# gillesdegottex/percivaltts

Measured on AMD Instinct MI355X. Metric: acoustic frames/sec per WGAN-GP critic+gen step, higher is better.
Workload: dtype f32

## Files before the change

### include/percival_hip.h

```cpp
#ifndef PERCIVAL_HIP_H
#define PERCIVAL_HIP_H

#include <stddef.h>
#include <stdint.h>

#ifdef __cplusplus
extern "C" {
#endif

#define PTTS_OK            0
#define PTTS_EINVAL       -1
#define PTTS_ELAUNCH      -2
#define PTTS_EWORKSPACE   -3
#define PTTS_EDEVICE      -4

#define PTTS_IN_NONE     0
#define PTTS_IN_LRELU    1
#define PTTS_IN_MASKMUL  2

#define PTTS_PAD_SAME    0
#define PTTS_PAD_CAUSAL  1

#define PTTS_ACT_NONE    0
#define PTTS_ACT_LRELU   1
#define PTTS_ACT_SIGMOID 2
#define PTTS_ACT_TANH    3

const char* ptts_version(void);
const char* ptts_device_arch(void);
const char* ptts_last_error(void);
int ptts_device_status(unsigned* word_out);
int ptts_device_status_clear(void);
unsigned* ptts_device_status_word(void);
int ptts_device_status_message(unsigned word, char* buf, size_t n);
int ptts_set_deterministic(int on);
int ptts_get_deterministic(void);
int ptts_set_bf16_products(int on);
int ptts_get_bf16_products(void);

int ptts_conv2d_fwd(const float* x, const float* w, const float* bias ,
                    const float* in_scale , const float* in_shift ,
                    const float* mask_src ,
                    float* y,
                    int B, int T, int F, int Cin, int Cout, int KT, int KF,
                    int dil_t, int pad_mode, int in_mode, float alpha, void* stream);

size_t ptts_conv2d_bwd_workspace_bytes(int B, int T, int F, int Cin, int Cout, int KT, int KF, int dil_t);
int ptts_conv2d_bwd(const float* dy, const float* x, const float* w,
                    const float* in_scale, const float* in_shift, const float* mask_src,
                    float* dx, float* dw, float* dbias, float* dscale, float* dshift,
                    void* workspace, size_t workspace_bytes,
                    int B, int T, int F, int Cin, int Cout, int KT, int KF,
                    int dil_t, int pad_mode, int in_mode, float alpha, void* stream);

int ptts_conv2d_bwd_partials(const float* dy, const float* x, const float* w, const float* mask_src,
                             float* dx, void* workspace, size_t workspace_bytes, int* nblocks_out,
                             int B, int T, int F, int Cin, int Cout, int KT, int KF,
                             int dil_t, int pad_mode, int in_mode, float alpha, void* stream);
typedef struct ptts_conv2d_reduce_desc {
    const float* partials;
    int nblocks, npart, nw, cout;
    float* dw; float* dbias;
} ptts_conv2d_reduce_desc;
int ptts_conv2d_reduce_grouped(const ptts_conv2d_reduce_desc* descs, int n, void* stream);

int ptts_conv2d_wide_supported(int F, int Cin, int Cout, int KT, int KF, int dil_t);
int ptts_conv2d_wide_fwd(const float* x, const float* w, const float* bias, const float* in_scale, const float* in_shift,
                         const float* mask_src, float* y, int B, int T, int F, int Cin, int Cout, int KT, int KF,
                         int dil_t, int pad_mode, int in_mode, float alpha, void* stream);
size_t ptts_conv2d_wide_bwd_workspace_bytes(int B, int T, int F, int Cin, int Cout, int KT, int KF, int dil_t);
int ptts_conv2d_wide_bwd_partials(const float* dy, const float* x, const float* w, const float* in_scale, const float* in_shift,
                                  const float* mask_src, float* dx, void* workspace, size_t workspace_bytes,
                                  int* nblocks_out, int* npart_out, int want_dw, int want_affine,
                                  int B, int T, int F, int Cin, int Cout, int KT, int KF,
                                  int dil_t, int pad_mode, int in_mode, float alpha, void* stream);

int ptts_conv2d_mfma_supported(int F, int Cin, int Cout, int KT, int KF, int dil_t);
size_t ptts_conv2d_mfma_table_bytes(int KT);
int ptts_conv2d_mfma_tables(const float* w, void* table_fwd, void* table_bwd, int KT, int KF, int Cin, int Cout,
                            int planes , void* stream);
int ptts_conv2d_mfma_tables_grouped(const float* const* w, void* const* table_fwd, void* const* table_bwd, int n, int planes,
                                    void* stream);
int ptts_conv2d_mfma_fwd(const void* x, const void* table, const float* bias, const float* in_scale, const float* in_shift,
                         const void* mask_src, const void* out_mask, void* y,
                         int B, int T, int F, int KT, int dil_t, int pad_t, int in_mode, float alpha,
                         int planes, int in_bf16, int out_bf16, void* stream);
int ptts_conv2d_mfma_fwd_stats_supported(int F, int dil_t, int in_mode);
int ptts_conv2d_mfma_fwd_stats(const float* x, const void* table, const float* bias, const float* in_scale, const float* in_shift,
                               float* y, int B, int T, int F, int KT, int pad_t, int in_mode, float alpha,
                               double* stats, int capacity_rows, int* nrows_out, void* stream);
size_t ptts_conv2d_mfma_wgrad_workspace_bytes(int B, int T);
int ptts_conv2d_mfma_wgrad_partials(const void* dy, const void* x, const void* mask_src, void* workspace,
                                    size_t workspace_bytes, int* nblocks_out, int* npart_out, int B, int T, int F,
                                    int KT, int dil_t, int pad_t, int in_mode, float alpha,
                                    int planes, int x_bf16, int dy_bf16, void* stream);
size_t ptts_conv2d_mfma_bwd_fused_workspace_bytes(int B, int T);
int ptts_conv2d_mfma_bwd_fused_supported(int F, int dil_t, int planes);
int ptts_conv2d_mfma_bwd_fused(const void* p, const void* q, const void* mask_src, const void* table, void* y,
                               void* workspace, size_t workspace_bytes, int* nblocks_out, int* npart_out,
                               int B, int T, int F, int KT, int pad_t, int kind, float alpha, void* stream);
int ptts_conv2d_mfma_bwd_fused_affine(const float* p, const float* q, const void* table, float* y, void* workspace, size_t workspace_bytes,
                                      int* nblocks_out, int* npart_out, int B, int T, int F, int KT, int pad_t, float alpha,
                                      const float* q_scale, const float* q_shift, void* stream);
int ptts_conv2d_mfma_debug(int flags, void* stamp_buf);

int ptts_conv2d_chain_supported(int F, int L, int Cin0, int C, int KT, int KF);
int ptts_conv2d_chain_blocks(int F, int L, int* origin, int* own_lo, int* own_hi, int cap);
int ptts_conv2d_chain_debug(void* stamp_buf);
size_t ptts_conv2d_chain_tables_bytes(void);
size_t ptts_conv2d_chain_partials_bytes(int L);
long long ptts_conv2d_chain_map_elems(int B, int T, int F);
int ptts_conv2d_chain_tables(const float* const* w, const float* const* b, void* tables, int L, int cin0, void* stream);
int ptts_conv2d_chain_fwd(const float* x0, long long ldx, const void* tables, void* maps, void* a_last,
                          int B, int T, int F, int L, float alpha, void* stream);
int ptts_conv2d_chain_bwd(const void* d_last, int d_bf16, const float* x0, long long ldx, const void* maps, const void* a_last,
                          const void* tables, float* partials, size_t partials_bytes, int* nblocks_out, int* npart_out,
                          int B, int T, int F, int L, int cin0, float alpha, void* stream);
int ptts_conv2d_chain_bwd_data(const void* d_last, int d_bf16, const void* maps, const void* a_last, const void* tables,
                               void* gmaps, float* g0, int B, int T, int F, int L, float alpha, void* stream);
int ptts_conv2d_chain_second(const float* u0, const void* gmaps, const void* maps, const void* a_last, const void* tables,
                             void* out, int out_bf16, float* partials, size_t partials_bytes, int* nblocks_out, int* npart_out,
                             int B, int T, int F, int L, int cin0, float alpha, void* stream);

int ptts_gemm(const float* A, const float* Bm, const float* bias, float* C,
              int M, int N, int K,
              int transA, long long lda, long long rows_per_seg, long long seg_stride,
              int transB, long long ldb, long long ldc,
              int in_mode, const float* in_scale, const float* in_shift, const float* mask_src,
              float alpha, int accumulate, const float* out_mask, float* colsum_b, void* stream);
// ... 370 lines not shown
```

### percivaltts_amd/csrc/conv2d.hip

```cpp
#include "common.h"
#include <cstdlib>

namespace ptts {

template <int C> struct VecIO;
template <> struct VecIO<1> {
    static __device__ __forceinline__ void ld(const float* p, float* v) { v[0] = p[0]; }
    static __device__ __forceinline__ void st(float* p, const float* v) { p[0] = v[0]; }
};
template <> struct VecIO<2> {
    static __device__ __forceinline__ void ld(const float* p, float* v) {
        float2 t = *reinterpret_cast<const float2*>(p); v[0] = t.x; v[1] = t.y; }
    static __device__ __forceinline__ void st(float* p, const float* v) {
        *reinterpret_cast<float2*>(p) = make_float2(v[0], v[1]); }
};
template <> struct VecIO<4> {
    static __device__ __forceinline__ void ld(const float* p, float* v) {
        float4 t = *reinterpret_cast<const float4*>(p); v[0] = t.x; v[1] = t.y; v[2] = t.z; v[3] = t.w; }
    static __device__ __forceinline__ void st(float* p, const float* v) {
        *reinterpret_cast<float4*>(p) = make_float4(v[0], v[1], v[2], v[3]); }
};

constexpr int CONV_THREADS = 256;

// ... 497 lines not shown
                    const float av = arow[(size_t)fq * CIN];
#pragma unroll
                    for (int kf = 0; kf < KF; ++kf) {
                        const int slot = (u + KF - 1 - kf) % KF;
                        if (PKO) {
#pragma unroll
                            for (int h = 0; h < HO; ++h)
                                accw2[kf][h] = pkfma(av, (f2){win[slot][2 * h], win[slot][2 * h + (PKO ? 1 : 0)]}, accw2[kf][h]);
                        } else {
#pragma unroll
                            for (int co = 0; co < COUT; ++co)
                                accw[kf][co] = fmaf(av, win[slot][co], accw[kf][co]);
                        }
                    }
                }
            }
        }
    }
    if (PKO) {
#pragma unroll
        for (int kf = 0; kf < KF; ++kf)
#pragma unroll
            for (int h = 0; h < HO; ++h) {
                accw[kf][2 * h] = accw2[kf][h].x;
                accw[kf][2 * h + (PKO ? 1 : 0)] = accw2[kf][h].y;
            }
    }
    float s_b[COUT];
#pragma unroll
    for (int co = 0; co < COUT; ++co) s_b[co] = 0.f;
    if (want_dw) {
        for (int idx = tid; idx < TT * F; idx += CONV_THREADS) {
            const int r = idx / F, f = idx - r * F;
            if (t0 + r >= T) break;
            float g[COUT];
            VecIO<COUT>::ld(dyt + ((size_t)(r + lo_t) * cols + f + LO_F) * COUT, g);
#pragma unroll
            for (int co = 0; co < COUT; ++co) s_b[co] += g[co];
        }
    }
    __syncthreads();

    float* red = smem;
    float* red2 = smem + (size_t)NGRP * NW;
    if (want_dw && grp < NGRP) {
#pragma unroll
        for (int kf = 0; kf < KF; ++kf)
#pragma unroll
            for (int co = 0; co < COUT; ++co)
                red[(size_t)grp * NW + ((rkt * KF + kf) * CIN + rci) * COUT + co] = accw[kf][co];
    }
    {
        const int wave = tid >> 6, lane = tid & 63;
#pragma unroll
        for (int co = 0; co < COUT; ++co) {
            const float v = wave_sum(s_b[co]);
            if (lane == 0) red2[wave * (COUT + 2 * CIN) + co] = v;
        }
#pragma unroll
        for (int ci = 0; ci < CIN; ++ci) {
            const float v1 = wave_sum(s_scale[ci]);
            const float v2 = wave_sum(s_shift[ci]);
            if (lane == 0) {
                red2[wave * (COUT + 2 * CIN) + COUT + ci] = v1;
                red2[wave * (COUT + 2 * CIN) + COUT + CIN + ci] = v2;
            }
        }
    }
    __syncthreads();
    float* out = partials + (size_t)(blockIdx.y * gridDim.x + blockIdx.x) * NPART;
    if (want_dw) {
        for (int j = tid; j < NW; j += CONV_THREADS) {
            float s = 0.f;
#pragma unroll
            for (int g = 0; g < NGRP; ++g) s += red[(size_t)g * NW + j];
            out[j] = s;
        }
    }
    if (tid < COUT + 2 * CIN) {
        float s = 0.f;
#pragma unroll
        for (int wv = 0; wv < CONV_THREADS / 64; ++wv) s += red2[wv * (COUT + 2 * CIN) + tid];
        out[NW + tid] = s;
    }
}

__global__ __launch_bounds__(256) void reduce_partials_kernel(const float* __restrict__ partials,
                                                              int nblocks, int npart,
                                                              float* __restrict__ dw, int nw,
                                                              float* __restrict__ dbias, int cout,
                                                              float* __restrict__ dscale,
                                                              float* __restrict__ dshift, int cin) {
    __shared__ double sh[4];
    const int j = blockIdx.x;
    double s = 0.0;
    for (int blk = threadIdx.x; blk < nblocks; blk += 256) s += (double)partials[(size_t)blk * npart + j];
    s = wave_sum(s);
    if ((threadIdx.x & 63) == 0) sh[threadIdx.x >> 6] = s;
    __syncthreads();
    if (threadIdx.x == 0) {
        const float v = (float)(sh[0] + sh[1] + sh[2] + sh[3]);
        if (j < nw) { if (dw) dw[j] = v; }
        else if (j < nw + cout) { if (dbias) dbias[j - nw] = v; }
        else if (j < nw + cout + cin) { if (dscale) dscale[j - nw - cout] = v; }
        else { if (dshift) dshift[j - nw - cout - cin] = v; }
    }
}

__device__ __forceinline__ float gen_in(const float* __restrict__ x, const float* __restrict__ in_scale,
                                        const float* __restrict__ in_shift,
                                        const float* __restrict__ mask_src, long long off, int c,
                                        int in_mode, float alpha) {
    float v = x[off];
    if (in_mode == PTTS_IN_LRELU) {
        if (in_scale) v = v * in_scale[c] + in_shift[c];
        v = lrelu(v, alpha);
    } else if (in_mode == PTTS_IN_MASKMUL) {
        v *= lrelu_d(mask_src[off], alpha);
    }
    return v;
}

__global__ void conv2d_fwd_generic(const float* __restrict__ x, const float* __restrict__ w,
                                   const float* __restrict__ bias, const float* __restrict__ in_scale,
                                   const float* __restrict__ in_shift, const float* __restrict__ mask_src,
                                   float* __restrict__ y, long long total, int T, int F, int Cin, int Cout,
                                   int KT, int KF, int dil_t, int pad_t, int in_mode, float alpha) {
    const int PF = (KF - 1) / 2;
    for (long long i = blockIdx.x * (long long)blockDim.x + threadIdx.x; i < total;
         i += (long long)gridDim.x * blockDim.x) {
        const int co = (int)(i % Cout);
        long long pix = i / Cout;
        const int f = (int)(pix % F);
        pix /= F;
        const int t = (int)(pix % T);
        const long long b = pix / T;
        float acc = bias ? bias[co] : 0.f;
        for (int kt = 0; kt < KT; ++kt) {
            const int tt = t + kt * dil_t - pad_t;
            if (tt < 0 || tt >= T) continue;
            for (int kf = 0; kf < KF; ++kf) {
                const int ff = f + kf - PF;
                if (ff < 0 || ff >= F) continue;
                const long long base = ((b * T + tt) * F + ff) * Cin;
                for (int ci = 0; ci < Cin; ++ci)
                    acc = fmaf(gen_in(x, in_scale, in_shift, mask_src, base + ci, ci, in_mode, alpha),
                               w[((kt * KF + kf) * Cin + ci) * Cout + co], acc);
            }
        }
        y[i] = acc;
    }
}

__global__ void conv2d_bwd_dx_generic(const float* __restrict__ dy, const float* __restrict__ x,
                                      const float* __restrict__ w, const float* __restrict__ in_scale,
                                      const float* __restrict__ in_shift, float* __restrict__ dx,
                                      long long total, int T, int F, int Cin, int Cout, int KT, int KF,
                                      int dil_t, int pad_t, int in_mode, float alpha) {
    const int PF = (KF - 1) / 2;
    for (long long i = blockIdx.x * (long long)blockDim.x + threadIdx.x; i < total;
         i += (long long)gridDim.x * blockDim.x) {
        const int ci = (int)(i % Cin);
        long long pix = i / Cin;
        const int f = (int)(pix % F);
        pix /= F;
        const int t = (int)(pix % T);
// ... 159 lines not shown

#define PTTS_CONV_CASES(M)                                                                    \
    M(1, 1, 3, 3) M(1, 2, 3, 3) M(1, 4, 3, 3) M(2, 1, 3, 3) M(2, 2, 3, 3) M(2, 4, 3, 3)       \
    M(4, 1, 3, 3) M(4, 2, 3, 3) M(4, 4, 3, 3)                                                 \
    M(1, 1, 5, 5) M(1, 2, 5, 5) M(1, 4, 5, 5) M(2, 1, 5, 5) M(2, 2, 5, 5) M(2, 4, 5, 5)       \
    M(4, 1, 5, 5) M(4, 2, 5, 5) M(4, 4, 5, 5)

}

using namespace ptts;

extern "C" int ptts_conv2d_fwd(const float* x, const float* w, const float* bias, const float* in_scale,
                               const float* in_shift, const float* mask_src, float* y, int B, int T, int F,
                               int Cin, int Cout, int KT, int KF, int dil_t, int pad_mode, int in_mode,
                               float alpha, void* stream) {
    PTTS_REQUIRE(x && w && y, "conv2d_fwd: null tensor");
    PTTS_REQUIRE(B > 0 && T > 0 && F > 0 && Cin > 0 && Cout > 0 && KT > 0 && KF > 0 && dil_t > 0,
                 "conv2d_fwd: bad dims B=%d T=%d F=%d Cin=%d Cout=%d KT=%d KF=%d dil=%d", B, T, F, Cin, Cout, KT, KF, dil_t);
    PTTS_REQUIRE(in_mode >= 0 && in_mode <= 2, "conv2d_fwd: bad in_mode %d", in_mode);
    PTTS_REQUIRE((in_scale == nullptr) == (in_shift == nullptr), "conv2d_fwd: scale/shift must come together");
    PTTS_REQUIRE(in_mode != PTTS_IN_MASKMUL || mask_src, "conv2d_fwd: MASKMUL needs mask_src");
    PTTS_REQUIRE(B <= 65535, "conv2d_fwd: B too large");
    hipStream_t st = (hipStream_t)stream;
    const ConvGeom g = geom(KT, dil_t, pad_mode);
#define FWD_LAUNCH(CI, CO, KTT, KFF, NRR, MK)                                                           \
    hipLaunchKernelGGL((conv2d_fwd_kernel<CI, CO, KTT, KFF, NRR, MK>), dim3(grid), dim3(CONV_THREADS), lds, \
                       st, x, w, bias, in_scale, in_shift, mask_src, y, T, F, tl.TT, tl.ntiles,             \
                       tl.ntiles * B, dil_t, g.pad_t, in_mode, alpha)
#define FWD_CASE(CI, CO, KTT, KFF)                                                                       \
    if (Cin == CI && Cout == CO && KT == KTT && KF == KFF) {                                             \
        const int nspr = (F + KFF - 1) / KFF;                                                            \
        const int cols = nspr * KFF + KFF - 1;                                                           \
        const Tile tl = pick_tile_fwd(T, F, KTT, KFF, dil_t, cols);                                      \
        const int rows = tl.TT + (KTT - 1) * dil_t;                                                      \
        const size_t in_fl = ((size_t)rows * cols * CI + 3) & ~(size_t)3;                                \
        const size_t lds = (in_fl + (size_t)tl.TT * F * CO) * sizeof(float);                             \
        const int nr = (tl.TT * nspr + CONV_THREADS - 1) / CONV_THREADS;                                 \
        if (tl.TT > 0 && lds <= 150 * 1024 && nr <= 2 && rows * cols <= NPF * CONV_THREADS) {            \
            int per_cu = (int)((150 * 1024) / lds);                                                      \
            if (per_cu > 4) per_cu = 4;                                                                  \
            long long grid = (long long)tl.ntiles * B;                                                   \
            if (grid > 256LL * per_cu) grid = 256LL * per_cu;                                            \
            const bool mk = in_mode == PTTS_IN_MASKMUL;                                                  \
            if (conv_use_mfma() && dil_t >= 1) {                                                         \
                if (mk) hipLaunchKernelGGL((conv2d_fwd_mfma_kernel<CI, CO, KTT, KFF, true, 2>), dim3(grid), dim3(CONV_THREADS), lds, st, x, w, bias, in_scale, in_shift, mask_src, y, T, F, tl.TT, tl.ntiles, tl.ntiles * B, dil_t, g.pad_t, in_mode, alpha); \
                else hipLaunchKernelGGL((conv2d_fwd_mfma_kernel<CI, CO, KTT, KFF, false, 2>), dim3(grid), dim3(CONV_THREADS), lds, st, x, w, bias, in_scale, in_shift, mask_src, y, T, F, tl.TT, tl.ntiles, tl.ntiles * B, dil_t, g.pad_t, in_mode, alpha); \
                return check_launch("conv2d_fwd_mfma");                                                  \
            }                                                                                            \
            if (nr == 1) { if (mk) FWD_LAUNCH(CI, CO, KTT, KFF, 1, true); else FWD_LAUNCH(CI, CO, KTT, KFF, 1, false); } \
            else { if (mk) FWD_LAUNCH(CI, CO, KTT, KFF, 2, true); else FWD_LAUNCH(CI, CO, KTT, KFF, 2, false); }         \
            return check_launch("conv2d_fwd");                                                           \
        }                                                                                                \
    }
    PTTS_CONV_CASES(FWD_CASE)
#undef FWD_CASE
#undef FWD_LAUNCH
    const long long total = (long long)B * T * F * Cout;
    const int blocks = (int)((total + 255) / 256 < 65536 ? (total + 255) / 256 : 65536);
    hipLaunchKernelGGL(conv2d_fwd_generic, dim3(blocks), dim3(256), 0, st, x, w, bias, in_scale, in_shift,
                       mask_src, y, total, T, F, Cin, Cout, KT, KF, dil_t, g.pad_t, in_mode, alpha);
    return check_launch("conv2d_fwd_generic");
}

namespace {
constexpr size_t WT_BYTES = 4096;
struct BwdPlan { bool fast; Tile tl; size_t lds; int npart; };
template <int CI, int CO, int KTT, int KFF>
BwdPlan plan_bwd(int T, int F, int dil_t) {
    BwdPlan p;
    const int nspr = (F + KFF - 1) / KFF;
    const int Fp = nspr * KFF;
    const size_t halo_row = (size_t)(Fp + KFF - 1) * CO * sizeof(float);
    const size_t fixed_row = (size_t)Fp * CI * sizeof(float) * 2;
    p.tl = pick_tile(T, F, KTT, KFF, dil_t, fixed_row, halo_row);
    p.lds = (size_t)p.tl.TT * fixed_row + (size_t)(p.tl.TT + (KTT - 1) * dil_t) * halo_row;
    constexpr int NW = KTT * KFF * CI * CO;
    constexpr int NGRP = CONV_THREADS / (KTT * CI);
    const size_t red = ((size_t)NGRP * NW + 4 * (CO + 2 * CI)) * sizeof(float);
    if (p.lds < red) p.lds = red;
    p.npart = NW + CO + 2 * CI;
    p.fast = p.lds <= 160 * 1024 - 256;
    return p;
}
}

extern "C" size_t ptts_conv2d_bwd_workspace_bytes(int B, int T, int F, int Cin, int Cout, int KT, int KF,
                                                  int dil_t) {
#define WS_CASE(CI, CO, KTT, KFF)                                                      \
    if (Cin == CI && Cout == CO && KT == KTT && KF == KFF) {                           \
        const BwdPlan p = plan_bwd<CI, CO, KTT, KFF>(T, F, dil_t);                     \
        if (p.fast) return WT_BYTES + (size_t)B * p.tl.ntiles * p.npart * sizeof(float); \
    }
    PTTS_CONV_CASES(WS_CASE)
#undef WS_CASE
    return 16;
}

static int conv2d_bwd_impl(const float* dy, const float* x, const float* w, const float* in_scale,
                           const float* in_shift, const float* mask_src, float* dx, float* dw,
                           float* dbias, float* dscale, float* dshift, void* workspace,
                           size_t workspace_bytes, int B, int T, int F, int Cin, int Cout, int KT, int KF,
                           int dil_t, int pad_mode, int in_mode, float alpha, void* stream, int partials_only,
                           int* nblocks_out) {
    PTTS_REQUIRE(dy && x && w, "conv2d_bwd: null tensor");
    PTTS_REQUIRE(B > 0 && T > 0 && F > 0 && Cin > 0 && Cout > 0 && KT > 0 && KF > 0 && dil_t > 0,
                 "conv2d_bwd: bad dims");
    PTTS_REQUIRE(in_mode >= 0 && in_mode <= 2, "conv2d_bwd: bad in_mode %d", in_mode);
    PTTS_REQUIRE((in_scale == nullptr) == (in_shift == nullptr), "conv2d_bwd: scale/shift must come together");
    PTTS_REQUIRE(in_mode != PTTS_IN_MASKMUL || mask_src, "conv2d_bwd: MASKMUL needs mask_src");
    PTTS_REQUIRE(!(in_mode == PTTS_IN_MASKMUL && dx), "conv2d_bwd: dx is not defined for MASKMUL (weight-only sweep)");
    PTTS_REQUIRE((dscale == nullptr) == (dshift == nullptr), "conv2d_bwd: dscale/dshift must come together");
    PTTS_REQUIRE(!dscale || (in_mode == PTTS_IN_LRELU && in_scale), "conv2d_bwd: dscale needs LRELU with scale/shift");
    PTTS_REQUIRE(B <= 65535, "conv2d_bwd: B too large");
    hipStream_t st = (hipStream_t)stream;
    const ConvGeom g = geom(KT, dil_t, pad_mode);
    const int want_dx = dx != nullptr, want_dw = (dw != nullptr || dbias != nullptr || partials_only), want_aff = dscale != nullptr;
    if (!want_dx && !want_dw && !want_aff) return PTTS_OK;
#define BWD_CASE(CI, CO, KTT, KFF)                                                                         \
    if (Cin == CI && Cout == CO && KT == KTT && KF == KFF) {                                               \
        const BwdPlan p = plan_bwd<CI, CO, KTT, KFF>(T, F, dil_t);                                         \
        if (p.fast) {                                                                                      \
            const int nblocks = B * p.tl.ntiles;                                                           \
            const size_t need = WT_BYTES + (size_t)nblocks * p.npart * sizeof(float);                      \
            if (!workspace || workspace_bytes < need) {                                                    \
                set_error("conv2d_bwd: workspace %zu < %zu", workspace_bytes, need);                       \
                return PTTS_EWORKSPACE;                                                                    \
            }                                                                                              \
            float* wt = (float*)workspace;                                                                 \
            float* parts = (float*)((char*)workspace + WT_BYTES);                                          \
            hipLaunchKernelGGL((conv2d_bwd_kernel<CI, CO, KTT, KFF>), dim3(p.tl.ntiles, B),                \
                               dim3(CONV_THREADS), p.lds, st, dy, x, w, in_scale, in_shift, mask_src, dx,  \
                               parts, (const float*)wt, want_dx, want_dw, want_aff, T, F, p.tl.TT, dil_t,  \
                               g.pad_t, in_mode, alpha);                                                   \
            int rc = check_launch("conv2d_bwd");                                                           \
            if (rc) return rc;                                                                             \
            if (nblocks_out) *nblocks_out = nblocks;                                                       \
            if ((want_dw || want_aff) && !partials_only) {                                                 \
                hipLaunchKernelGGL(reduce_partials_kernel, dim3(p.npart), dim3(256), 0, st,                \
                                   (const float*)parts, nblocks, p.npart, want_dw ? dw : nullptr,          \
                                   KTT * KFF * CI * CO, want_dw ? dbias : nullptr, CO, dscale, dshift, CI);\
                rc = check_launch("conv2d_bwd_reduce");                                                    \
            }                                                                                              \
            return rc;                                                                                     \
        }                                                                                                  \
    }
    PTTS_CONV_CASES(BWD_CASE)
#undef BWD_CASE
    PTTS_REQUIRE(!partials_only, "conv2d_bwd_partials: this shape has no tiled kernel (workspace_bytes == 16): use ptts_conv2d_bwd");
    const long long npix = (long long)B * T * F;
    if (want_dx) {
        const long long total = npix * Cin;
        const int blocks = (int)((total + 255) / 256 < 65536 ? (total + 255) / 256 : 65536);
        hipLaunchKernelGGL(conv2d_bwd_dx_generic, dim3(blocks), dim3(256), 0, st, dy, x, w, in_scale, in_shift,
                           dx, total, T, F, Cin, Cout, KT, KF, dil_t, g.pad_t, in_mode, alpha);
        int rc = check_launch("conv2d_bwd_dx_generic");
        if (rc) return rc;
    }
    if (want_dw || want_aff) {
        const int nw = KT * KF * Cin * Cout;
        const int nblk = nw + Cout + (want_aff ? 2 * Cin : 0);
        hipLaunchKernelGGL(conv2d_bwd_w_generic, dim3(nblk), dim3(256), 0, st, dy, x, w, in_scale, in_shift,
                           mask_src, want_dw ? dw : nullptr, want_dw ? dbias : nullptr, dscale, dshift, npix, T,
                           F, Cin, Cout, KT, KF, dil_t, g.pad_t, in_mode, alpha);
        return check_launch("conv2d_bwd_w_generic");
    }
    return PTTS_OK;
}

extern "C" int ptts_conv2d_bwd(const float* dy, const float* x, const float* w, const float* in_scale,
                               const float* in_shift, const float* mask_src, float* dx, float* dw,
                               float* dbias, float* dscale, float* dshift, void* workspace,
                               size_t workspace_bytes, int B, int T, int F, int Cin, int Cout, int KT, int KF,
                               int dil_t, int pad_mode, int in_mode, float alpha, void* stream) {
    return conv2d_bwd_impl(dy, x, w, in_scale, in_shift, mask_src, dx, dw, dbias, dscale, dshift, workspace, workspace_bytes,
                           B, T, F, Cin, Cout, KT, KF, dil_t, pad_mode, in_mode, alpha, stream, 0, nullptr);
}

extern "C" int ptts_conv2d_bwd_partials(const float* dy, const float* x, const float* w, const float* mask_src,
                                        float* dx, void* workspace, size_t workspace_bytes, int* nblocks_out,
                                        int B, int T, int F, int Cin, int Cout, int KT, int KF,
                                        int dil_t, int pad_mode, int in_mode, float alpha, void* stream) {
    PTTS_REQUIRE(nblocks_out, "conv2d_bwd_partials: nblocks_out is NULL");
    return conv2d_bwd_impl(dy, x, w, nullptr, nullptr, mask_src, dx, nullptr, nullptr, nullptr, nullptr, workspace,
                           workspace_bytes, B, T, F, Cin, Cout, KT, KF, dil_t, pad_mode, in_mode, alpha, stream, 1, nblocks_out);
}

constexpr int RG_MAX = 16;
struct ReduceGroupArgs {
    int n;
    int col_begin[RG_MAX + 1];
    const float* partials[RG_MAX]; int nblocks[RG_MAX], npart[RG_MAX], nw[RG_MAX], ncout[RG_MAX];
    float* dw[RG_MAX]; float* dbias[RG_MAX];
};

constexpr int RG_COLS = 64, RG_ROWS = 4, RG_SLAB = 128;
__global__ __launch_bounds__(RG_COLS * RG_ROWS) void conv2d_reduce_grouped_kernel(ReduceGroupArgs a) {
    __shared__ double sh[RG_ROWS][RG_COLS];
    int gi = 0;
    while ((int)blockIdx.x >= a.col_begin[gi + 1]) ++gi;
    const int cx = threadIdx.x & (RG_COLS - 1), ry = threadIdx.x / RG_COLS;
    const int npart = a.npart[gi], nblocks = a.nblocks[gi], ncols = a.nw[gi] + a.ncout[gi];
    const int nchunks = (ncols + RG_COLS - 1) / RG_COLS, r = blockIdx.x - a.col_begin[gi];
    const int slab = r / nchunks, j = (r - slab * nchunks) * RG_COLS + cx;
    const int row_end = min(nblocks, (slab + 1) * RG_SLAB);
    const float* p = a.partials[gi] + j;
    double s0 = 0.0, s1 = 0.0, s2 = 0.0, s3 = 0.0;
    if (j < ncols) {
        int blk = slab * RG_SLAB + ry;
        for (; blk + 3 * RG_ROWS < row_end; blk += 4 * RG_ROWS) {
            const float v0 = p[(size_t)blk * npart], v1 = p[(size_t)(blk + RG_ROWS) * npart];
            const float v2 = p[(size_t)(blk + 2 * RG_ROWS) * npart], v3 = p[(size_t)(blk + 3 * RG_ROWS) * npart];
            s0 += (double)v0; s1 += (double)v1; s2 += (double)v2; s3 += (double)v3;
        }
        for (; blk < row_end; blk += RG_ROWS) s0 += (double)p[(size_t)blk * npart];
    }
    sh[ry][cx] = (s0 + s1) + (s2 + s3);
// ... 34 lines not shown
```

Measured before the change: 5.116 million.

## Add persistent conv2d backward kernel with register prefetch of next tile

Adds a persistent-grid conv2d backward kernel that loops over tiles and prefetches the next tile's dy/x into registers while computing the current one. Weight gradients stay in registers across tiles, so each block writes a single partial row, and the reduction kernel sees far fewer blocks. A host planner picks the tile height, occupancy from register and LDS limits, and the dW segment split. It is enabled by default through an env toggle. Risks include register pressure from the prefetch arrays, lower occupancy, and a larger workspace requirement.

Result: no change. 5.107 million (-0.2%).

```diff
diff --git a/include/percival_hip.h b/include/percival_hip.h
--- a/include/percival_hip.h
+++ b/include/percival_hip.h
@@ -45,6 +45,8 @@
                     int B, int T, int F, int Cin, int Cout, int KT, int KF,
                     int dil_t, int pad_mode, int in_mode, float alpha, void* stream);
 
+int ptts_set_conv2d_bwd_persistent(int on);
+int ptts_set_conv2d_bwd_grid(int max_workgroups);
 size_t ptts_conv2d_bwd_workspace_bytes(int B, int T, int F, int Cin, int Cout, int KT, int KF, int dil_t);
 int ptts_conv2d_bwd(const float* dy, const float* x, const float* w,
                     const float* in_scale, const float* in_shift, const float* mask_src,
diff --git a/percivaltts_amd/csrc/conv2d.hip b/percivaltts_amd/csrc/conv2d.hip
--- a/percivaltts_amd/csrc/conv2d.hip
+++ b/percivaltts_amd/csrc/conv2d.hip
@@ -603,6 +603,341 @@
 #pragma unroll
         for (int wv = 0; wv < CONV_THREADS / 64; ++wv) s += red2[wv * (COUT + 2 * CIN) + tid];
         out[NW + tid] = s;
+    }
+}
+
+constexpr int NPD = 7;
+constexpr int NPX = 5;
+
+template <int CIN, int COUT>
+struct BwdPrefetch {
+    float d[NPD][COUT];
+    float v[NPX][CIN];
+    float m[NPX][CIN];
+    unsigned okx;
+};
+
+template <int CIN, int COUT>
+__device__ __forceinline__ void bwd_prefetch(BwdPrefetch<CIN, COUT>& pf, const float* __restrict__ dy,
+                                             const float* __restrict__ x, const float* __restrict__ mask_src,
+                                             long long img, int T, int F, int rows, int cols, int t_org, int f_org,
+                                             int TT, int Fp, int t0, bool need_x, bool mask) {
+    const int total = rows * cols;
+#pragma unroll
+    for (int u = 0; u < NPD; ++u) {
+        const int idx = threadIdx.x + u * CONV_THREADS;
+        const int r = idx / cols, c = idx - r * cols;
+        const int t = t_org + r, f = f_org + c;
+#pragma unroll
+        for (int c2 = 0; c2 < COUT; ++c2) pf.d[u][c2] = 0.f;
+        if (idx < total && t >= 0 && t < T && f >= 0 && f < F)
+            VecIO<COUT>::ld(dy + (img + (long long)t * F + f) * COUT, pf.d[u]);
+    }
+    pf.okx = 0u;
+    if (need_x) {
+        const int totx = TT * Fp;
+#pragma unroll
+        for (int u = 0; u < NPX; ++u) {
+            const int idx = threadIdx.x + u * CONV_THREADS;
+            const int r = idx / Fp, f = idx - r * Fp;
+            const int t = t0 + r;
+#pragma unroll
+            for (int c2 = 0; c2 < CIN; ++c2) { pf.v[u][c2] = 0.f; pf.m[u][c2] = 0.f; }
+            if (idx < totx && t < T && f < F) {
+                const long long off = (img + (long long)t * F + f) * CIN;
+                VecIO<CIN>::ld(x + off, pf.v[u]);
+                if (mask) VecIO<CIN>::ld(mask_src + off, pf.m[u]);
+                pf.okx |= 1u << u;
+            }
+        }
+    }
+}
+
+template <int CIN, int COUT>
+__device__ __forceinline__ void bwd_commit(const BwdPrefetch<CIN, COUT>& pf, float* __restrict__ dyt,
+                                           float* __restrict__ at, float* __restrict__ xt, int totd, int totx,
+                                           bool need_x, const float* __restrict__ in_scale,
+                                           const float* __restrict__ in_shift, int in_mode, float alpha) {
+#pragma unroll
+    for (int u = 0; u < NPD; ++u) {
+        const int idx = threadIdx.x + u * CONV_THREADS;
+        if (idx < totd) VecIO<COUT>::st(dyt + (size_t)idx * COUT, pf.d[u]);
+    }
+    if (!need_x) return;
+#pragma unroll
+    for (int u = 0; u < NPX; ++u) {
+        const int idx = threadIdx.x + u * CONV_THREADS;
+        if (idx >= totx) continue;
+        float a[CIN];
+#pragma unroll
+        for (int c2 = 0; c2 < CIN; ++c2) a[c2] = pf.v[u][c2];
+        if (xt) VecIO<CIN>::st(xt + (size_t)idx * CIN, a);
+        if ((pf.okx >> u) & 1u) {
+            if (in_mode == PTTS_IN_LRELU) {
+#pragma unroll
+                for (int c2 = 0; c2 < CIN; ++c2) {
+                    float p = a[c2];
+                    if (in_scale) p = p * in_scale[c2] + in_shift[c2];
+                    a[c2] = lrelu(p, alpha);
+                }
+            } else if (in_mode == PTTS_IN_MASKMUL) {
+#pragma unroll
+                for (int c2 = 0; c2 < CIN; ++c2) a[c2] *= lrelu_d(pf.m[u][c2], alpha);
+            }
+        }
+        VecIO<CIN>::st(at + (size_t)idx * CIN, a);
+    }
+}
+
+template <int CIN, int COUT, int KT, int KF>
+__global__ __launch_bounds__(CONV_THREADS) void conv2d_bwd_persistent_kernel(
+    const float* __restrict__ dy, const float* __restrict__ x, const float* __restrict__ w,
+    const float* __restrict__ in_scale, const float* __restrict__ in_shift,
+    const float* __restrict__ mask_src, float* __restrict__ dx, float* __restrict__ partials,
+    int want_dx, int want_dw, int want_affine,
+    int T, int F, int TT, int ntiles_t, int ntiles, int nseg, int seglen, int dil_t, int pad_t, int in_mode, float alpha) {
+    extern __shared__ __attribute__((aligned(16))) float smem[];
+    constexpr int P = KF;
+    constexpr int PF = (KF - 1) / 2;
+    constexpr int LO_F = (KF - 1) - PF;
+    constexpr int NW = KT * KF * CIN * COUT;
+    constexpr int NPART = NW + COUT + 2 * CIN;
+    const int nspr = (F + P - 1) / P;
+    const int Fp = nspr * P;
+    const int cols = Fp + KF - 1;
+    const int halo_t = (KT - 1) * dil_t;
+    const int lo_t = halo_t - pad_t;
+    const int rows = TT + halo_t;
+
+    float* dyt = smem;
+    float* at = dyt + (((size_t)rows * cols * COUT + 3) & ~(size_t)3);
+    float* xt = at + (((size_t)TT * Fp * CIN + 3) & ~(size_t)3);
+    const int tid = threadIdx.x;
+    const bool need_x = want_dw || want_affine || (want_dx && in_mode == PTTS_IN_LRELU);
+    const bool mask = in_mode == PTTS_IN_MASKMUL;
+
+    double t_scale[CIN], t_shift[CIN], t_b[COUT];
+#pragma unroll
+    for (int c = 0; c < CIN; ++c) { t_scale[c] = 0.0; t_shift[c] = 0.0; }
+#pragma unroll
+    for (int co = 0; co < COUT; ++co) t_b[co] = 0.0;
+    constexpr int NROLE = KT * CIN;
+    constexpr int NGRP = CONV_THREADS / NROLE;
+    constexpr bool PKO = (COUT % 2 == 0);
+    constexpr int HO = PKO ? COUT / 2 : 1;
+    float accw[KF][COUT];
+    f2 accw2[KF][HO];
+#pragma unroll
+    for (int kf = 0; kf < KF; ++kf) {
+#pragma unroll
+        for (int co = 0; co < COUT; ++co) accw[kf][co] = 0.f;
+#pragma unroll
+        for (int h = 0; h < HO; ++h) accw2[kf][h] = (f2){0.f, 0.f};
+    }
+    const int grp = tid / NROLE;
+    const int role = tid - grp * NROLE;
+    const int rkt = role / CIN, rci = role - rkt * CIN;
+
+    int tile = blockIdx.x;
+    BwdPrefetch<CIN, COUT> pf;
+    if (tile < ntiles) {
+        const int b = tile / ntiles_t, t0 = (tile - b * ntiles_t) * TT;
+        bwd_prefetch<CIN, COUT>(pf, dy, x, mask_src, (long long)b * T * F, T, F, rows, cols, t0 - lo_t, -LO_F, TT, Fp, t0, need_x, mask);
+    }
+    while (tile < ntiles) {
+        const int b = tile / ntiles_t, t0 = (tile - b * ntiles_t) * TT;
+        const long long img = (long long)b * T * F;
+        bwd_commit<CIN, COUT>(pf, dyt, at, want_affine ? xt : nullptr, rows * cols, TT * Fp, need_x, in_scale, in_shift, in_mode, alpha);
+        __syncthreads();
+        const int next = tile + gridDim.x;
+        if (next < ntiles) {
+            const int nb = next / ntiles_t, nt0 = (next - nb * ntiles_t) * TT;
+            bwd_prefetch<CIN, COUT>(pf, dy, x, mask_src, (long long)nb * T * F, T, F, rows, cols, nt0 - lo_t, -LO_F, TT, Fp, nt0, need_x, mask);
+        }
+
+        if (want_dx || want_affine) {
+            const int nstrips = TT * nspr;
+            for (int s = tid; s < nstrips; s += CONV_THREADS) {
+                const int r = s / nspr;
+                const int fs = (s - r * nspr) * P;
+                const int t = t0 + r;
+                if (t >= T) continue;
+                constexpr bool PKI = (COUT % 2 == 0);
+                constexpr int HO2 = PKI ? COUT / 2 : 1;
+                float da[P][CIN];
+                f2 da2[P][CIN];
+#pragma unroll
+                for (int p = 0; p < P; ++p) {
+#pragma unroll
+                    for (int ci = 0; ci < CIN; ++ci) { da[p][ci] = 0.f; da2[p][ci] = (f2){0.f, 0.f}; }
+                }
+#pragma unroll 1
+                for (int kt = 0; kt < KT; ++kt) {
+                    const float* row = dyt + ((size_t)(r + (KT - 1 - kt) * dil_t) * cols + fs) * COUT;
+#pragma unroll
+                    for (int j = 0; j < P + KF - 1; ++j) {
+                        float g[COUT];
+                        VecIO<COUT>::ld(row + j * COUT, g);
+#pragma unroll
+                        for (int kf = 0; kf < KF; ++kf) {
+                            const int p = j - (KF - 1 - kf);
+                            if (p < 0 || p >= P) continue;
+                            const float* wk = w + ((kt * KF + kf) * CIN) * COUT;
+                            if (PKI) {
+                                const f2* wk2 = reinterpret_cast<const f2*>(wk);
+#pragma unroll
+                                for (int ci = 0; ci < CIN; ++ci)
+#pragma unroll
+                                    for (int h = 0; h < HO2; ++h)
+                                        da2[p][ci] = __builtin_elementwise_fma((f2){g[2 * h], g[2 * h + (PKI ? 1 : 0)]}, wk2[ci * HO2 + h], da2[p][ci]);
+                            } else {
+#pragma unroll
+                                for (int ci = 0; ci < CIN; ++ci)
+#pragma unroll
+                                    for (int co = 0; co < COUT; ++co)
+                                        da[p][ci] = fmaf(g[co], wk[ci * COUT + co], da[p][ci]);
+                            }
+                        }
+                    }
+                }
+                if (PKI) {
+#pragma unroll
+                    for (int p = 0; p < P; ++p)
+#pragma unroll
+                        for (int ci = 0; ci < CIN; ++ci) da[p][ci] = da2[p][ci].x + da2[p][ci].y;
+                }
+                const float* arow = at + ((size_t)r * Fp + fs) * CIN;
+                const float* xrow = xt + ((size_t)r * Fp + fs) * CIN;
+                float* dxo = dx + (img + (long long)t * F + fs) * CIN;
+#pragma unroll
+                for (int p = 0; p < P; ++p) {
+                    if (fs + p >= F) continue;
+                    float o[CIN];
+                    if (in_mode == PTTS_IN_LRELU) {
+                        float a[CIN];
+                        VecIO<CIN>::ld(arow + p * CIN, a);
+#pragma unroll
+                        for (int ci = 0; ci < CIN; ++ci) {
+                            const float gd = da[p][ci] * (a[ci] > 0.f ? 1.f : alpha);
+                            o[ci] = in_scale ? gd * in_scale[ci] : gd;
+                            da[p][ci] = gd;
+                        }
+                        if (want_affine) {
+                            float xr[CIN];
+                            VecIO<CIN>::ld(xrow + p * CIN, xr);
+#pragma unroll
+                            for (int ci = 0; ci < CIN; ++ci) {
+                                t_shift[ci] += (double)da[p][ci];
+                                t_scale[ci] += (double)da[p][ci] * (double)xr[ci];
+                            }
+                        }
+                    } else {
+#pragma unroll
+                        for (int ci = 0; ci < CIN; ++ci) o[ci] = da[p][ci];
+                    }
+                    if (want_dx) VecIO<CIN>::st(dxo + p * CIN, o);
+                }
+            }
+        }
+
+        const int nrows = min(TT, T - t0);
+        if (want_dw && grp < NGRP) {
+            const int nitems = nrows * nseg;
+            for (int it = grp; it < nitems; it += NGRP) {
+                const int r = it / nseg;
+                const int fb = (it - r * nseg) * seglen;
+                const int fe = min(Fp, fb + seglen);
+                const float* drow = dyt + ((size_t)(r + (KT - 1 - rkt) * dil_t) * cols + fb) * COUT;
+                const float* arow = at + ((size_t)r * Fp + fb) * CIN + rci;
+                float win[KF][COUT];
+#pragma unroll
+                for (int k = 0; k < KF - 1; ++k) VecIO<COUT>::ld(drow + k * COUT, win[k]);
+                for (int f0 = 0; f0 < fe - fb; f0 += KF) {
+#pragma unroll
+                    for (int u = 0; u < KF; ++u) {
+                        const int fq = f0 + u;
+                        VecIO<COUT>::ld(drow + (size_t)(fq + KF - 1) * COUT, win[(u + KF - 1) % KF]);
+                        const float av = arow[(size_t)fq * CIN];
+#pragma unroll
+                        for (int kf = 0; kf < KF; ++kf) {
+                            const int slot = (u + KF - 1 - kf) % KF;
+                            if (PKO) {
+#pragma unroll
+                                for (int h = 0; h < HO; ++h)
+                                    accw2[kf][h] = pkfma(av, (f2){win[slot][2 * h], win[slot][2 * h + (PKO ? 1 : 0)]}, accw2[kf][h]);
+                            } else {
+#pragma unroll
+                                for (int co = 0; co < COUT; ++co)
+                                    accw[kf][co] = fmaf(av, win[slot][co], accw[kf][co]);
+                            }
+                        }
+                    }
+                }
+            }
+        }
+        if (want_dw) {
+            for (int idx = tid; idx < nrows * F; idx += CONV_THREADS) {
+                const int r = idx / F, f = idx - r * F;
+                float g[COUT];
+                VecIO<COUT>::ld(dyt + ((size_t)(r + lo_t) * cols + f + LO_F) * COUT, g);
+#pragma unroll
+                for (int co = 0; co < COUT; ++co) t_b[co] += (double)g[co];
+            }
+        }
+        __syncthreads();
+        tile = next;
+    }
+
+    if (PKO) {
+#pragma unroll
+        for (int kf = 0; kf < KF; ++kf)
+#pragma unroll
+            for (int h = 0; h < HO; ++h) {
+                accw[kf][2 * h] = accw2[kf][h].x;
+                accw[kf][2 * h + (PKO ? 1 : 0)] = accw2[kf][h].y;
+            }
+    }
+    float* red = smem;
+    double* red2 = reinterpret_cast<double*>(smem + (((size_t)NGRP * NW + 1) & ~(size_t)1));
+    if (want_dw && grp < NGRP) {
+#pragma unroll
+        for (int kf = 0; kf < KF; ++kf)
+#pragma unroll
+            for (int co = 0; co < COUT; ++co)
+                red[(size_t)grp * NW + ((rkt * KF + kf) * CIN + rci) * COUT + co] = accw[kf][co];
+    }
+    {
+        const int wave = tid >> 6, lane = tid & 63;
+#pragma unroll
+        for (int co = 0; co < COUT; ++co) {
+            const double v = wave_sum(t_b[co]);
+            if (lane == 0) red2[wave * (COUT + 2 * CIN) + co] = v;
+        }
+#pragma unroll
+        for (int ci = 0; ci < CIN; ++ci) {
+            const double v1 = wave_sum(t_scale[ci]);
+            const double v2 = wave_sum(t_shift[ci]);
+            if (lane == 0) {
+                red2[wave * (COUT + 2 * CIN) + COUT + ci] = v1;
+                red2[wave * (COUT + 2 * CIN) + COUT + CIN + ci] = v2;
+            }
+        }
+    }
+    __syncthreads();
+    float* out = partials + (size_t)blockIdx.x * NPART;
+    if (want_dw) {
+        for (int j = tid; j < NW; j += CONV_THREADS) {
+            double s = 0.0;
+#pragma unroll
+            for (int g = 0; g < NGRP; ++g) s += (double)red[(size_t)g * NW + j];
+            out[j] = (float)s;
+        }
+    }
+    if (tid < COUT + 2 * CIN) {
+        double s = 0.0;
+#pragma unroll
+        for (int wv = 0; wv < CONV_THREADS / 64; ++wv) s += red2[wv * (COUT + 2 * CIN) + tid];
+        out[NW + tid] = (float)s;
     }
 }
 
@@ -928,6 +1263,97 @@
     p.fast = p.lds <= 160 * 1024 - 256;
     return p;
 }
+
+int g_bwd_persistent = -1;
+int g_bwd_grid = 0;
+int bwd_persistent_on() {
+    if (g_bwd_persistent < 0) { const char* e = getenv("PTTS_CONV_BWD_PERSISTENT"); g_bwd_persistent = e ? (atoi(e) != 0 ? 1 : 0) : 1; }
+    return g_bwd_persistent;
+}
+constexpr int PERS_MAX_PER_CU = 4;
+constexpr size_t PERS_LDS_PER_CU = 150 * 1024;
+
+template <int CI, int CO, int KTT, int KFF>
+int pers_k_regs() {
+    static const int k = [] {
+        int kk = CI * CO <= 2 ? 4 : (CI * CO <= 4 ? 3 : 2);
+        hipFuncAttributes a;
+        if (hipFuncGetAttributes(&a, reinterpret_cast<const void*>(&conv2d_bwd_persistent_kernel<CI, CO, KTT, KFF>)) == hipSuccess && a.numRegs > 0)
+            kk = 512 / ((a.numRegs + 7) & ~7);
+        else
+            (void)hipGetLastError();
+        return kk < 1 ? 1 : (kk > PERS_MAX_PER_CU ? PERS_MAX_PER_CU : kk);
+    }();
+    return k;
+}
+
+struct PersPlan { bool ok; int TT, ntiles_t; size_t lds; int k, nseg, seglen; };
+
+static void pick_segments(int TT, int nspr, int KF, int ngrp, int* nseg, int* seglen) {
+    long long best = -1;
+    for (int ns = 1; ns <= nspr; ++ns) {
+        const int sl = (nspr + ns - 1) / ns, real = (nspr + sl - 1) / sl;
+        const long long rounds = ((long long)TT * real + ngrp - 1) / ngrp;
+        const long long cost = rounds * (sl * KF + KF - 1);
+        if (best < 0 || cost < best) { best = cost; *nseg = real; *seglen = sl * KF; }
+    }
+}
+
+template <int CI, int CO, int KTT, int KFF>
+PersPlan plan_bwd_pers(int B, int T, int F, int dil_t) {
+    PersPlan best{false, 0, 0, 0, 1, 1, KFF};
+    const int nspr = (F + KFF - 1) / KFF;
+    const int Fp = nspr * KFF, cols = Fp + KFF - 1;
+    const int halo = (KTT - 1) * dil_t;
+    constexpr int NW = KTT * KFF * CI * CO;
+    constexpr int NGRP = CONV_THREADS / (KTT * CI);
+    const size_t red = ((size_t)NGRP * NW + 1 + 8 * (CO + 2 * CI)) * sizeof(float);
+    static const int forced = [] { const char* e = getenv("PTTS_CONV_BWD_TT"); return e ? atoi(e) : 0; }();
+    const int kregs = pers_k_regs<CI, CO, KTT, KFF>();
+    double best_score = -1.0;
+    for (int TT = 1; TT <= 128; ++TT) {
+        if ((long long)(TT + halo) * cols > NPD * CONV_THREADS || (long long)TT * Fp > NPX * CONV_THREADS) break;
+        if (forced > 0 && TT != forced) continue;
+        size_t lds = ((((size_t)(TT + halo) * cols * CO + 3) & ~(size_t)3) + 2 * (((size_t)TT * Fp * CI + 3) & ~(size_t)3)) * sizeof(float);
+        if (lds < red) lds = red;
+        if (lds > lds_budget() && best.ok) break;
+        if (lds > PERS_LDS_PER_CU) break;
+        int k = (int)(PERS_LDS_PER_CU / lds);
+        if (k > kregs) k = kregs;
+        const int ntiles_t = (T + TT - 1) / TT;
+        const long long tiles = (long long)ntiles_t * B, G = 256LL * k;
+        const double balance = tiles <= G ? 1.0 : (double)tiles / (double)(((tiles + G - 1) / G) * G);
+        const int strips = TT * nspr;
+        const int rounds = (strips + CONV_THREADS - 1) / CONV_THREADS;
+        const double lane_eff = (double)strips / (rounds * CONV_THREADS);
+        const double row_eff = (double)T / ((double)ntiles_t * TT);
+        const double halo_eff = (double)TT / (TT + halo);
+        const double score = lane_eff * row_eff * (0.75 + 0.25 * halo_eff) * balance;
+        if (score > best_score + 1e-9) {
+            best_score = score;
+            best = PersPlan{true, TT, ntiles_t, lds, k, 1, KFF};
+        }
+    }
+    if (best.ok) pick_segments(best.TT, nspr, KFF, NGRP, &best.nseg, &best.seglen);
+    return best;
+}
+
+static int pers_grid(const PersPlan& q, int B) {
+    const long long tiles = (long long)q.ntiles_t * B, G = 256LL * q.k;
+    if (g_bwd_grid > 0) return (int)(g_bwd_grid < G ? g_bwd_grid : G);
+    return (int)(tiles < G ? tiles : G);
+}
+}
+
+extern "C" int ptts_set_conv2d_bwd_persistent(int on) {
+    const int prev = bwd_persistent_on();
+    g_bwd_persistent = on ? 1 : 0;
+    return prev;
+}
+extern "C" int ptts_set_conv2d_bwd_grid(int max_workgroups) {
+    const int prev = g_bwd_grid;
+    g_bwd_grid = max_workgroups > 0 ? max_workgroups : 0;
+    return prev;
 }
 
 extern "C" size_t ptts_conv2d_bwd_workspace_bytes(int B, int T, int F, int Cin, int Cout, int KT, int KF,
@@ -935,7 +1361,12 @@
 #define WS_CASE(CI, CO, KTT, KFF)                                                      \
     if (Cin == CI && Cout == CO && KT == KTT && KF == KFF) {                           \
         const BwdPlan p = plan_bwd<CI, CO, KTT, KFF>(T, F, dil_t);                     \
-        if (p.fast) return WT_BYTES + (size_t)B * p.tl.ntiles * p.npart * sizeof(float); \
+        if (p.fast) {                                                                  \
+             \
+            size_t rows = (size_t)B * p.tl.ntiles;                                     \
+            if (rows < 256 * (size_t)PERS_MAX_PER_CU) rows = 256 * (size_t)PERS_MAX_PER_CU; \
+            return WT_BYTES + rows * p.npart * sizeof(float);                          \
+        }                                                                              \
     }
     PTTS_CONV_CASES(WS_CASE)
 #undef WS_CASE
@@ -966,7 +1397,9 @@
     if (Cin == CI && Cout == CO && KT == KTT && KF == KFF) {                                               \
         const BwdPlan p = plan_bwd<CI, CO, KTT, KFF>(T, F, dil_t);                                         \
         if (p.fast) {                                                                                      \
-            const int nblocks = B * p.tl.ntiles;                                                           \
+            PersPlan q{false, 0, 0, 0, 1, 1, KFF};                                                         \
+            if (bwd_persistent_on()) q = plan_bwd_pers<CI, CO, KTT, KFF>(B, T, F, dil_t);                  \
+            const int nblocks = q.ok ? pers_grid(q, B) : B * p.tl.ntiles;                                  \
             const size_t need = WT_BYTES + (size_t)nblocks * p.npart * sizeof(float);                      \
             if (!workspace || workspace_bytes < need) {                                                    \
                 set_error("conv2d_bwd: workspace %zu < %zu", workspace_bytes, need);                       \
@@ -974,10 +1407,16 @@
             }                                                                                              \
             float* wt = (float*)workspace;                                                                 \
             float* parts = (float*)((char*)workspace + WT_BYTES);                                          \
-            hipLaunchKernelGGL((conv2d_bwd_kernel<CI, CO, KTT, KFF>), dim3(p.tl.ntiles, B),                \
-                               dim3(CONV_THREADS), p.lds, st, dy, x, w, in_scale, in_shift, mask_src, dx,  \
-                               parts, (const float*)wt, want_dx, want_dw, want_aff, T, F, p.tl.TT, dil_t,  \
-                               g.pad_t, in_mode, alpha);                                                   \
+            if (q.ok)                                                                                      \
+                hipLaunchKernelGGL((conv2d_bwd_persistent_kernel<CI, CO, KTT, KFF>), dim3(nblocks),        \
+                                   dim3(CONV_THREADS), q.lds, st, dy, x, w, in_scale, in_shift, mask_src,  \
+                                   dx, parts, want_dx, want_dw, want_aff, T, F, q.TT, q.ntiles_t,          \
+                                   q.ntiles_t * B, q.nseg, q.seglen, dil_t, g.pad_t, in_mode, alpha);      \
+            else                                                                                           \
+                hipLaunchKernelGGL((conv2d_bwd_kernel<CI, CO, KTT, KFF>), dim3(p.tl.ntiles, B),            \
+                                   dim3(CONV_THREADS), p.lds, st, dy, x, w, in_scale, in_shift, mask_src,  \
+                                   dx, parts, (const float*)wt, want_dx, want_dw, want_aff, T, F, p.tl.TT, \
+                                   dil_t, g.pad_t, in_mode, alpha);                                        \
             int rc = check_launch("conv2d_bwd");                                                           \
             if (rc) return rc;                                                                             \
             if (nblocks_out) *nblocks_out = nblocks;                                                       \
```
